# lvjiahui/DRT

Hardware: AMD Instinct MI355X
Metric: M camera-rays/s (forward+backward) on 50k-tri mesh, 72 views (higher is better)
Workload: dtype f32 traversal + f64 shading/gradients; 1 GPU; horse_vh.ply x4 (1 midpoint subdivision) = 50248 tris / 25126 verts, 72 turntable views, 1024x1024 rays/view, LBVH rebuilt every step, forward+ray_loss+backward+all-reduce+SGD; targets=horse_scan.ply, mode=dropin, hip_graph=False, outputs_recycled=True, ray_binding=True, views_per_gpu=72, views_per_call=72

## Files before the change

### drt_amd/csrc/drt_pipeline.hip

```cpp
#include "drt_device.h"
#include "drt_trace_kernel.h"
#include "drt_pathsink.h"


struct Ray64 {
    double* o;
    double* d;
};
struct Pipe {
    RayList r0, r1, r2;
    unsigned* count;
    unsigned* valid;
    int32_t* redo;
};




__device__ __forceinline__ void write_dead(int64_t i, double* out_ori, double* out_dir, uint8_t* mask, int32_t* face2) {
    const d3 z{0.0, 0.0, 0.0};
    store_d3(out_ori, i, z);
    store_d3(out_dir, i, z);
    mask[3 * i] = 0; mask[3 * i + 1] = 0; mask[3 * i + 2] = 0;
    face2[i] = -1;
// ... 15 lines not shown
        po[lane] = zero; pd[lane] = zero;
        if (lane < 32) { po[64 + lane] = zero; pd[64 + lane] = zero; }
        if (lane < 12) reinterpret_cast<F4*>(mask + 3 * i0)[lane] = zero;
        if (lane >= 16 && lane < 32) reinterpret_cast<F4*>(face2 + i0)[lane - 16] = ones;
    }
    if (lane >= 32 && lane < 48) reinterpret_cast<F4*>(face1 + i0)[lane - 32] = ones;
}

struct RasterIn {
    ViewModel* views;
    int mode;
    unsigned long long* zbuf;
    uint32_t* zmask;
    int32_t* gen_list;
    int img_w, img_h;
    int pending;
    int no_tree;
};
constexpr int32_t kFacePending = -2;

struct CullShared {
    unsigned tmp[kPathWaves + 1];
    uint8_t flag[kPathBlock];
    int slot[kPathBlock];
};

template <bool FUSED>
__device__ __forceinline__ void cull_patch(unsigned patch, bool prefilled, CullShared& sh, const Node4Q* __restrict__ nodes, int n_tris,
                                           const double* __restrict__ origin, const double* __restrict__ dir,
                                           const uint8_t* __restrict__ valid, int64_t n, double* __restrict__ out_ori,
                                           double* __restrict__ out_dir, uint8_t* __restrict__ mask,
                                           int32_t* __restrict__ face1, int32_t* __restrict__ face2, const Pipe& p, int tile_w, const RasterIn& rz) {
    unsigned* s_tmp = sh.tmp;
    uint8_t* s_flag = sh.flag;
    int* s_slot = sh.slot;
    const bool dead_writes = !FUSED && !prefilled;
    const int tid = threadIdx.x;
    const bool raster = rz.views != nullptr;
    const int vt = ((tid & 63) >> 4) * 64 + (tid >> 6) * 16 + (tid & 15);
    const unsigned patches_per_row = tile_w > 0 ? (unsigned)tile_w / 64u : 1u;
    {
        int64_t i = (int64_t)patch * kPathBlock + tid;
        unsigned y = 0, x = 0;
        if (tile_w > 0) {
            const unsigned prow = patch / patches_per_row;
            y = 4u * prow + (unsigned)(tid >> 6); x = 64u * (patch - prow * patches_per_row) + (unsigned)(tid & 63);
            i = (int64_t)y * tile_w + x;
        }
        if (raster && rz.mode == DRT_GRID_TRUST) {
            const unsigned view = y / (unsigned)rz.img_h;
            if (rz.views[view].ok && rz.views[view].all) {
                const int64_t row0 = i - (int64_t)(tid >> 6) * tile_w - (tid & 63);
                unsigned any = 0;
                for (int r = 0; r < 4; ++r) {
                    const int64_t g = (row0 + (int64_t)r * tile_w) >> 6;
                    any |= rz.zmask[g >> 5] >> (g & 31);
                }
                if (!(any & 1u)) {
                    if (dead_writes) write_dead_row<FUSED>(i - (tid & 63), tid & 63, out_ori, out_dir, mask, face1, face2);
                    return;
                }
            }
        }
        bool cand = false, generic = false;
        int32_t face = -1;
        unsigned clear_bit = 0;
        f3 o{0.f, 0.f, 0.f}, d{0.f, 0.f, 1.f};
        if (i < n) {
            unsigned long long key = kRasterEmpty;
            bool trusted = false;
            unsigned view = 0;
            if (raster) {
                view = y / (unsigned)rz.img_h;
                trusted = rz.mode == DRT_GRID_TRUST && rz.views[view].ok && rz.views[view].all;
                const unsigned word = rz.zmask[i >> 11], bit = 1u << ((i >> 6) & 31);
                if (word & bit) {
                    const int64_t zs = raster_slot(x, y, (unsigned)tile_w);
                    key = rz.zbuf[zs];
                    if (key != kRasterEmpty) rz.zbuf[zs] = kRasterEmpty;
                    clear_bit = bit;
                }
            }
            if (trusted) {
                if (key != kRasterEmpty && (!FUSED || valid[i])) {
                    o = to_f32(load_d3(origin, i)); d = to_f32(load_d3(dir, i));
                    cand = true;
                    face = (int32_t)(uint32_t)key;
                }
            } else if (!FUSED || valid[i]) {
                const d3 o64 = load_d3(origin, i), d64 = load_d3(dir, i);
                o = to_f32(o64); d = to_f32(d64);
                bool verified = false;
                if (raster) {
                    ViewModel& vm = rz.views[view];
                    verified = vm.ok && view_verify(vm, o64, d64, (double)x, (double)(y - view * (unsigned)rz.img_h));
                    if (!verified && vm.all) __hip_atomic_store(&vm.all, 0, __ATOMIC_RELAXED, __HIP_MEMORY_SCOPE_AGENT);
                }
                if (verified) {
                    cand = key != kRasterEmpty;
                    face = (int32_t)(uint32_t)key;
                } else {
                    cand = n_tris > 0 && (rz.no_tree || hits_top_boxes(nodes, o, d));
                    generic = cand;
                }
            } else if (raster && rz.mode == DRT_GRID_ESTABLISH) {
                ViewModel& vm = rz.views[view];
                if (vm.all && !(vm.ok && view_verify(vm, load_d3(origin, i), load_d3(dir, i), (double)x, (double)(y - view * (unsigned)rz.img_h))))
                    __hip_atomic_store(&vm.all, 0, __ATOMIC_RELAXED, __HIP_MEMORY_SCOPE_AGENT);
            }
        }
        const bool live = i < n;
        if (!dead_writes) {
        } else if (tile_w > 0 && __ballot(cand || !live) == 0ull) {
            write_dead_row<FUSED>(i - (tid & 63), tid & 63, out_ori, out_dir, mask, face1, face2);
        } else if (live && !cand) {
            face1[i] = -1;
            write_dead(i, out_ori, out_dir, mask, face2);
        }
        const int any_cand = __syncthreads_or(cand ? 1 : 0);
        if (clear_bit && (tid & 63) == 0) atomicAnd(&rz.zmask[i >> 11], ~clear_bit);
        if (!any_cand) return;
        int slot;
        if (tile_w > 0) {
            s_flag[vt] = cand ? 1 : 0;
            __syncthreads();
            s_slot[tid] = block_push(s_flag[tid] != 0, &p.count[0], s_tmp);
            __syncthreads();
            slot = s_slot[vt];
            __syncthreads();
        } else {
            slot = block_push(cand, &p.count[0], s_tmp);
        }
        if (slot >= 0) {
            p.r0.idx[slot] = (int32_t)i; store_ray32(p.r0.ray, slot, o, d);
            if (raster) p.r0.face[slot] = generic && rz.pending ? kFacePending : face;
        }
        if (raster && __syncthreads_or(generic ? 1 : 0)) {
            const int g = block_push(generic, &p.count[3], s_tmp);
            if (g >= 0) rz.gen_list[g] = slot;
        }
    }
}

template <bool FUSED>
__global__ void __launch_bounds__(kPathBlock, 8) k_cull(const Node4Q* __restrict__ nodes, int n_tris, const double* __restrict__ origin, const double* __restrict__ dir,
                                                      const uint8_t* __restrict__ valid, int64_t n, double* __restrict__ out_ori,
                                                      double* __restrict__ out_dir, uint8_t* __restrict__ mask,
                                                      int32_t* __restrict__ face1, int32_t* __restrict__ face2, Pipe p, int tile_w, RasterIn rz,
                                                      bool prefilled ) {
    __shared__ CullShared sh;
    cull_patch<FUSED>(blockIdx.x, prefilled, sh, nodes, n_tris, origin, dir, valid, n, out_ori, out_dir, mask, face1, face2, p, tile_w, rz);
}

struct StageFace {
    StageMem m;
    int32_t face[kStageCap];
};
template <bool FUSED>
__global__ void __launch_bounds__(kPathBlock) k_cull_listed(const uint32_t* __restrict__ patches, const unsigned* __restrict__ n_patches,
                                                           const Node4Q* __restrict__ nodes, int n_tris, const double* __restrict__ origin, const double* __restrict__ dir,
                                                           const uint8_t* __restrict__ valid, int64_t n, double* __restrict__ out_ori,
                                                           double* __restrict__ out_dir, uint8_t* __restrict__ mask,
                                                           int32_t* __restrict__ face1, int32_t* __restrict__ face2, Pipe p, int tile_w, RasterIn rz,
                                                           PathCtx c, bool direct, bool prefilled, Ray64 park) {
    __shared__ CullShared sh;
    __shared__ StageFace st;
    stage_init(st.m);
    const int tid = threadIdx.x, wave = tid >> 6, lane = tid & 63;
    const int vt = ((tid & 63) >> 4) * 64 + (tid >> 6) * 16 + (tid & 15);
    const unsigned ppr = (unsigned)tile_w / 64u;
    const RayList dst = direct ? p.r1 : p.r0;
    unsigned* const dst_count = direct ? &p.count[1] : &p.count[0];
    auto flush = [&]() {
        const unsigned cnt = st.m.n;
        if (tid == 0) st.m.base = cnt ? atomicAdd(dst_count, cnt) : 0u;
        __syncthreads();
        const unsigned base = st.m.base;
        for (unsigned k = tid; k < cnt; k += kPathBlock) { dst.idx[base + k] = st.m.idx[k]; if (!direct) dst.face[base + k] = st.face[k]; }
        for (unsigned k = tid; k < 6u * cnt; k += kPathBlock) dst.ray[6 * (int64_t)base + k] = st.m.ray[k];
        __syncthreads();
        if (tid == 0) st.m.n = 0u;
        __syncthreads();
    };
    unsigned n_hits = 0;
    const unsigned count = *n_patches;
    for (unsigned k = blockIdx.x; k < count; k += gridDim.x) {
        const unsigned patch = patches[k];
        const unsigned prow = patch / ppr;
        const unsigned y = 4u * prow + (unsigned)wave, x = 64u * (patch - prow * ppr) + (unsigned)lane;
        const unsigned view = y / (unsigned)rz.img_h;
        if (!(rz.views[view].ok && rz.views[view].all)) {
            cull_patch<FUSED>(patch, true, sh, nodes, n_tris, origin, dir, valid, n, out_ori, out_dir, mask, face1, face2, p, tile_w, rz);
            __syncthreads();
            continue;
        }
        const int64_t i = (int64_t)y * tile_w + x;
        unsigned long long key = kRasterEmpty;
        const unsigned word = rz.zmask[i >> 11], bit = 1u << ((i >> 6) & 31);
        if (word & bit) {
            const int64_t zs = raster_slot(x, y, (unsigned)tile_w);
            key = rz.zbuf[zs];
            if (key != kRasterEmpty) rz.zbuf[zs] = kRasterEmpty;
        }
        const bool cand = key != kRasterEmpty && (!FUSED || valid[i]);
        bool push = cand;
        f3 o{0.f, 0.f, 0.f}, d{0.f, 0.f, 1.f};
        if (cand) {
            if (direct) {
                const int32_t f1 = (int32_t)(uint32_t)key;
                face1[i] = f1;
                d3 v0, v1, v2;
                int32_t vid[3];
                Bounce b;
                load_tri64(c, f1, v0, v1, v2, vid);
                bounce_forward(load_d3(origin, i), load_d3(dir, i), v0, v1, v2, c.ior_ext, c.ior_int, b);
                push = !b.tir;
                o = to_f32(b.new_o); d = to_f32(b.wt);
                if (push && park.o) { store_d3(park.o, i, b.new_o); store_d3(park.d, i, b.wt); }
                if (!push && !FUSED) { if (prefilled) face2[i] = -1; else write_dead(i, out_ori, out_dir, mask, face2); }
                ++n_hits;
            } else {
                o = to_f32(load_d3(origin, i)); d = to_f32(load_d3(dir, i));
            }
        }
        sh.flag[vt] = push ? 1 : 0;
        __syncthreads();
        if ((word & bit) && lane == 0) atomicAnd(&rz.zmask[i >> 11], ~bit);
        const bool mine = sh.flag[tid] != 0;
        const unsigned long long bm = __ballot(mine);
        if (lane == 0) sh.tmp[wave] = (unsigned)__popcll(bm);
        __syncthreads();
        unsigned before = 0, tot = 0;
        for (int w = 0; w < kPathWaves; ++w) { const unsigned cw = sh.tmp[w]; if (w < wave) before += cw; tot += cw; }
        sh.slot[tid] = mine ? (int)(before + (unsigned)__popcll(bm & ((1ull << lane) - 1ull))) : -1;
        __syncthreads();
        if (push) {
            const unsigned slot = st.m.n + (unsigned)sh.slot[vt];
            st.m.idx[slot] = (int32_t)i;
            float* e = st.m.ray + 6 * slot;
            e[0] = o.x; e[1] = o.y; e[2] = o.z; e[3] = d.x; e[4] = d.y; e[5] = d.z;
            st.face[slot] = (int32_t)(uint32_t)key;
        }
        __syncthreads();
        if (tid == 0) st.m.n += tot;
        __syncthreads();
        if (st.m.n > kStageCap - kPathBlock) flush();
    }
    flush();
    if (direct) {
        unsigned h = n_hits;
        for (int off = 32; off >= 1; off >>= 1) h += __shfl_xor(h, off);
        if (lane == 0 && h) atomicAdd(&p.count[17], h);
    }
}

__global__ void __launch_bounds__(kPathBlock) k_patch_list(unsigned n_patches, int tile_w, RasterIn rz, uint32_t* __restrict__ list, unsigned* count) {
    __shared__ unsigned s_tmp[kPathWaves + 1];
    const unsigned patch = blockIdx.x * kPathBlock + threadIdx.x;
    bool take = false;
    if (patch < n_patches) {
        const unsigned ppr = (unsigned)tile_w / 64u, prow = patch / ppr;
        const unsigned view = (4u * prow) / (unsigned)rz.img_h;
        take = true;
        if (rz.views[view].ok && rz.views[view].all) {
            const int64_t row0 = (int64_t)(4u * prow) * tile_w + 64u * (patch - prow * ppr);
            unsigned any = 0;
            for (int r = 0; r < 4; ++r) {
                const int64_t g = (row0 + (int64_t)r * tile_w) >> 6;
                any |= rz.zmask[g >> 5] >> (g & 31);
            }
            take = (any & 1u) != 0;
        }
    }
    const int slot = block_push(take, count, s_tmp);
    if (slot >= 0) list[slot] = patch;
}

template <bool FUSED>
__global__ void __launch_bounds__(kPathBlock) k_shade1(PathCtx c, const double* __restrict__ origin, const double* __restrict__ dir,
                                                        double* __restrict__ out_ori, double* __restrict__ out_dir, uint8_t* __restrict__ mask,
                                                        int32_t* __restrict__ face1, int32_t* __restrict__ face2, Pipe p,
                                                        bool prefilled , Ray64 r64) {
    __shared__ StageMem stage;
    stage_init(stage);
    const unsigned n0 = p.count[0];
    const unsigned per_block = ((n0 + gridDim.x - 1) / gridDim.x + kPathBlock - 1) / kPathBlock * kPathBlock;
    const unsigned first = blockIdx.x * per_block, last = min(n0, first + per_block);
    for (unsigned base = first; base < last; base += kPathBlock) {
        const unsigned k = base + threadIdx.x;
        bool ok = false;
        int64_t i = 0;
        f3 o2{0.f, 0.f, 0.f}, d2{0.f, 0.f, 1.f};
        if (k < n0) {
            i = p.r0.idx[k];
            const int32_t f1 = p.r0.face[k];
            if (f1 != kFacePending) face1[i] = f1;
            if (f1 >= 0) {
                d3 v0, v1, v2;
                int32_t vid[3];
                Bounce b;
                load_tri64(c, f1, v0, v1, v2, vid);
                bounce_forward(load_d3(origin, i), load_d3(dir, i), v0, v1, v2, c.ior_ext, c.ior_int, b);
                ok = !b.tir;
                o2 = to_f32(b.new_o); d2 = to_f32(b.wt);
                if (ok && r64.o) { store_d3(r64.o, i, b.new_o); store_d3(r64.d, i, b.wt); }
            }
            if (!ok && !FUSED && f1 != kFacePending) { if (prefilled) face2[i] = -1; else write_dead(i, out_ori, out_dir, mask, face2); }
        }
        stage_push(stage, ok, (int32_t)i, o2, d2, p.r1, &p.count[1]);
    }
    stage_flush(stage, p.r1, &p.count[1]);
}

template <bool FUSED>
__global__ void __launch_bounds__(kTraceBlock) k_gen_late(PathCtx c, const double* __restrict__ origin, const double* __restrict__ dir,
                                                          double* __restrict__ out_ori, double* __restrict__ out_dir, uint8_t* __restrict__ mask,
                                                          int32_t* __restrict__ face1, int32_t* __restrict__ face2, Pipe p,
                                                          const int32_t* __restrict__ gen_list, bool prefilled, Ray64 r64) {
    __shared__ int32_t lds[kStackFast][kTraceBlock];
    const unsigned n = p.count[3];
    if (n == 0) return;
    Stack st = make_stack(lds, c.tc);
    for (unsigned k = blockIdx.x * kTraceBlock + threadIdx.x; k < n; k += gridDim.x * kTraceBlock) {
        const int32_t slot = gen_list[k];
        if (p.r0.face[slot] != kFacePending) continue;
        const int64_t i = p.r0.idx[slot];
        const float* e = p.r0.ray + 6 * (int64_t)slot;
        const Hit h = traverse<false>(c.tc.nodes, c.tc.tris, c.tc.n_tris, f3{e[0], e[1], e[2]}, f3{e[3], e[4], e[5]}, st);
        p.r0.face[slot] = h.face;
        face1[i] = h.face;
        bool ok = false;
        if (h.face >= 0) {
            d3 v0, v1, v2;
            int32_t vid[3];
            Bounce b;
            load_tri64(c, h.face, v0, v1, v2, vid);
            bounce_forward(load_d3(origin, i), load_d3(dir, i), v0, v1, v2, c.ior_ext, c.ior_int, b);
            ok = !b.tir;
            if (ok) {
                const unsigned s1 = atomicAdd(&p.count[1], 1u);
                p.r1.idx[s1] = (int32_t)i;
                store_ray32(p.r1.ray, (int)s1, to_f32(b.new_o), to_f32(b.wt));
                if (r64.o) { store_d3(r64.o, i, b.new_o); store_d3(r64.d, i, b.wt); }
            }
        }
        if (!ok && !FUSED) { if (prefilled) face2[i] = -1; else write_dead(i, out_ori, out_dir, mask, face2); }
    }
}

template <bool FUSED>
__global__ void __launch_bounds__(kPathBlock) k_shade2(PathCtx c, const double* __restrict__ origin, const double* __restrict__ dir,
                                                        double* __restrict__ out_ori, double* __restrict__ out_dir, uint8_t* __restrict__ mask,
                                                        const int32_t* __restrict__ face1, int32_t* __restrict__ face2, Pipe p,
                                                        bool parked ) {
    __shared__ StageMem stage;
    stage_init(stage);
    const unsigned n1 = p.count[1];
    const unsigned per_block = ((n1 + gridDim.x - 1) / gridDim.x + kPathBlock - 1) / kPathBlock * kPathBlock;
    const unsigned first = blockIdx.x * per_block, last = min(n1, first + per_block);
    for (unsigned base = first; base < last; base += kPathBlock) {
        const unsigned k = base + threadIdx.x;
        bool ok = false;
        int64_t i = 0;
        f3 o3{0.f, 0.f, 0.f}, d3f{0.f, 0.f, 1.f};
        if (k < n1) {
            i = p.r1.idx[k];
            const int32_t f2 = p.r1.face[k];
            if (f2 >= 0) {
                d3 v0, v1, v2;
                int32_t vid[3];
                Bounce b;
                d3 o2, d2;
                if (parked) {
                    o2 = load_d3(out_ori, i); d2 = load_d3(out_dir, i);
                } else {
                    load_tri64(c, face1[i], v0, v1, v2, vid);
                    bounce_forward(load_d3(origin, i), load_d3(dir, i), v0, v1, v2, c.ior_ext, c.ior_int, b);
                    o2 = b.new_o; d2 = b.wt;
                }
                load_tri64(c, f2, v0, v1, v2, vid);
                bounce_forward(o2, d2, v0, v1, v2, c.ior_ext, c.ior_int, b);
                ok = !b.tir;
                if (ok) {
                    o3 = to_f32(b.new_o); d3f = to_f32(b.wt);
                    face2[i] = f2;
                    if (!FUSED) {
                        store_d3(out_ori, i, b.new_o);
                        store_d3(out_dir, i, b.wt);
                        mask[3 * i] = 1; mask[3 * i + 1] = 1; mask[3 * i + 2] = 1;
                    }
                }
            }
            if (!ok) { if (FUSED) face2[i] = -1; else write_dead(i, out_ori, out_dir, mask, face2); }
        }
        stage_push(stage, ok, (int32_t)i, o3, d3f, p.r2, &p.count[2]);
    }
    stage_flush(stage, p.r2, &p.count[2]);
}

__global__ void __launch_bounds__(kPathBlock) k_finish(double* __restrict__ out_ori, double* __restrict__ out_dir, uint8_t* __restrict__ mask,
                                                        int32_t* __restrict__ face2, Pipe p, int64_t chunk_base, int32_t* __restrict__ valid_idx) {
    __shared__ StageMem stage;
    stage_init(stage);
    const RayList out{valid_idx, nullptr, nullptr};
    const unsigned n2 = p.count[2];
    const unsigned per_block = ((n2 + gridDim.x - 1) / gridDim.x + kPathBlock - 1) / kPathBlock * kPathBlock;
// ... 577 lines not shown

static int ensure_queues(drt_scene::Sub& w, int64_t n, bool fused, bool mega = false) {
    if (fused && mega && n > w.ray64_cap) {
        (void)hipFree(w.ray64); w.ray64 = nullptr; w.ray64_cap = 0;
        HIP_TRY(hipMalloc(&w.ray64, sizeof(double) * 6 * n));
        w.ray64_cap = n;
    }
    if (n > w.q_cap) {
        for (int k = 0; k < 3; ++k) {
            (void)hipFree(w.q_idx[k]); (void)hipFree(w.q_ray[k]); (void)hipFree(w.q_face[k]);
            w.q_idx[k] = nullptr; w.q_ray[k] = nullptr; w.q_face[k] = nullptr;
        }
        w.q_cap = 0;
        for (int k = 0; k < 3; ++k) {
            HIP_TRY(hipMalloc(&w.q_idx[k], sizeof(int32_t) * n));
            HIP_TRY(hipMalloc(&w.q_ray[k], sizeof(float) * 6 * n));
            HIP_TRY(hipMalloc(&w.q_face[k], sizeof(int32_t) * n));
        }
        (void)hipFree(w.redo); w.redo = nullptr;
        HIP_TRY(hipMalloc(&w.redo, sizeof(int32_t) * n));
        (void)hipFree(w.gen_list); w.gen_list = nullptr;
        HIP_TRY(hipMalloc(&w.gen_list, sizeof(int32_t) * n));
        w.q_cap = n;
    }
    if (fused && n > w.fused_cap) {
        (void)hipFree(w.tmp_face1); (void)hipFree(w.tmp_face2);
        w.tmp_face1 = w.tmp_face2 = nullptr; w.fused_cap = 0;
        HIP_TRY(hipMalloc(&w.tmp_face1, sizeof(int32_t) * n));
        HIP_TRY(hipMalloc(&w.tmp_face2, sizeof(int32_t) * n));
        w.fused_cap = n;
    }
    return DRT_OK;
}

static Pipe pipe_of(const drt_scene* s, const drt_scene::Sub& w) {
    return Pipe{RayList{w.q_idx[0], w.q_ray[0], w.q_face[0]}, RayList{w.q_idx[1], w.q_ray[1], w.q_face[1]},
                RayList{w.q_idx[2], w.q_ray[2], w.q_face[2]}, w.qcount, s->vcount, w.redo};
}

struct Plan { int64_t size; int count; int streams; };
static Plan plan_call(const drt_scene* s, int64_t n_rays, int tile_w, int tile_h) {
    int64_t unit = 256;
    if (tile_w >= 64 && tile_w % 64 == 0) unit = 4 * (int64_t)tile_w;
    if (unit > 256 && tile_h >= 4 && tile_h % 4 == 0 && n_rays % ((int64_t)tile_w * tile_h) == 0) unit = (int64_t)tile_w * tile_h;
    int64_t count = (n_rays + s->chunk_rays - 1) / s->chunk_rays;
    const int64_t by_min = n_rays / s->min_sub_rays;
    const int64_t most = (int64_t)s->n_sub * s->sub_per_stream;
    const int64_t want = by_min < most ? by_min : most;
    if (want > count) count = want;
    if (count < 1) count = 1;
    int64_t size = (n_rays + count - 1) / count;
    size = (size + unit - 1) / unit * unit;
    count = (n_rays + size - 1) / size;
    Plan pl;
    pl.size = size; pl.count = (int)count; pl.streams = count < s->n_sub ? (int)count : s->n_sub;
    if (s->prof_serial) pl.streams = 1;
    return pl;
}

__global__ void k_store_models(const ViewModel* __restrict__ work, ViewModel* __restrict__ cache, int n) {
    const int v = blockIdx.x * blockDim.x + threadIdx.x;
    if (v >= n) return;
    ViewModel m = work[v];
    m.all = (m.ok && m.all) ? 1 : 0;
    m.ok = m.all;
    cache[v] = m;
}

static bool raster_on(const drt_scene* s, int64_t n, int tile_w, int tile_h) {
    if (!s->use_raster || s->n_faces <= 0 || tile_w < 64 || tile_w % 64 != 0 || tile_h < 4 || tile_h % 4 != 0) return false;
    const int64_t image = (int64_t)tile_w * tile_h;
    return n > 0 && n % image == 0 && n / image <= 65535;
}

constexpr int kIntPreOri = 1 << 16, kIntPreDir = 1 << 17, kIntPreMask = 1 << 18, kIntMask = kIntPreOri | kIntPreDir | kIntPreMask;
extern "C++" {
template <bool FUSED>
static int launch_chunk(drt_scene* s, drt_scene::Sub& w, hipStream_t st, const PathCtx& pc, const Pipe& p, const double* o, const double* d, const uint8_t* valid,
                        int64_t n, double* out_ori, double* out_dir, uint8_t* mask, int32_t* face1, int32_t* face2, int tile_w, int tile_h,
                        int grid_mode, ViewModel* grid_cache ,
                        hipStream_t aux , int64_t chunk_base, int32_t* valid_idx,
                        bool* n_finished ,
                        int32_t* seed2 = nullptr ) {
    if (n_finished) *n_finished = false;
    const bool sparse_faces = (grid_mode & DRT_GRID_SPARSE_FACES) != 0;
    const bool pre_ori = (grid_mode & kIntPreOri) != 0, pre_dir = (grid_mode & kIntPreDir) != 0, pre_mask = (grid_mode & kIntPreMask) != 0;
    const bool all_verified = (grid_mode & DRT_GRID_ALL_VERIFIED) != 0 && (grid_mode & 3) == DRT_GRID_TRUST && grid_cache;
    grid_mode &= 3;
    const int gs = 8 * s->n_cu;
    if (tile_w < 64 || tile_w % 64 != 0 || n % (4 * (int64_t)tile_w) != 0) tile_w = 0;
    RasterIn rz{nullptr, 0, nullptr, nullptr, nullptr, 0, 0, 0, 0};
    const bool mega = s->mega_max_rays > 0 && n <= s->mega_max_rays && n_finished != nullptr;
    const Ray64 r64 = !mega ? Ray64{nullptr, nullptr} : (FUSED ? Ray64{w.ray64, w.ray64 + 3 * n} : Ray64{out_ori, out_dir});
    bool late_fill = false;
    hipStream_t fs = s->prof_serial ? st : s->build_stream;
    {
        hipStreamCaptureStatus cs = hipStreamCaptureStatusNone;
        if (fs != st && hipStreamIsCapturing(st, &cs) == hipSuccess && cs != hipStreamCaptureStatusNone) fs = aux ? aux : st;
    }
    const int64_t image = (int64_t)tile_w * tile_h;
    if (raster_on(s, n, tile_w, tile_h)) {
        const int n_views = (int)(n / image);
        int rc = ensure_raster(s, w, n, n_views, st);
        if (rc) return rc;
        if (!grid_cache) grid_mode = DRT_GRID_NONE;
        if (!FUSED && grid_mode == DRT_GRID_TRUST) {
            late_fill = s->fill_overlap;
            if (!late_fill) {
                StageTimer t(s, st, kStageFill);
                if (!pre_ori) (void)hipMemsetAsync(out_ori, 0, sizeof(double) * 3 * n, st);
                if (!pre_dir) (void)hipMemsetAsync(out_dir, 0, sizeof(double) * 3 * n, st);
                if (!pre_mask) (void)hipMemsetAsync(mask, 0, 3 * n, st);
            }
            if (!sparse_faces) { (void)hipMemsetAsync(face1, 0xFF, sizeof(int32_t) * n, st); (void)hipMemsetAsync(face2, 0xFF, sizeof(int32_t) * n, st); }
        }
        if (late_fill && mega) {
            if (fs != st && aux) fs = aux;
            if (fs != st) { HIP_TRY(hipEventRecord(w.fill_fork, st)); HIP_TRY(hipStreamWaitEvent(fs, w.fill_fork, 0)); }
            { StageTimer tf(s, fs, kStageFill);
              if (!pre_ori) (void)hipMemsetAsync(out_ori, 0, sizeof(double) * 3 * n, fs);
              if (!pre_dir) (void)hipMemsetAsync(out_dir, 0, sizeof(double) * 3 * n, fs);
              if (!pre_mask) (void)hipMemsetAsync(mask, 0, 3 * n, fs); }
            if (fs != st) HIP_TRY(hipEventRecord(w.fill_join, fs));
        }
        StageTimer t(s, st, kStageRaster);
        rc = launch_raster(s, w, st, o, d, n_views, tile_w, tile_h, grid_mode == DRT_GRID_TRUST ? grid_cache : nullptr);
        if (rc) return rc;
        rz = RasterIn{w.vmodel, grid_mode, w.zbuf, w.zmask, w.gen_list, tile_w, tile_h, all_verified ? 1 : 0, all_verified ? 1 : 0};
    }
    const bool pre_any = pre_ori || pre_dir || pre_mask;
    if (pre_any && !late_fill) HIP_TRY(hipStreamWaitEvent(st, s->prefill_done, 0));
    const bool tree_late = all_verified && rz.views != nullptr;
    if (!tree_late) { int rc = wait_build(s, st); if (rc) return rc; }
    const bool direct = s->cull_direct && rz.views && grid_mode == DRT_GRID_TRUST && !mega && n >= s->cull_direct_min_rays;
    const bool park = !FUSED && !mega && rz.views && grid_mode == DRT_GRID_TRUST && pre_ori && pre_dir && pre_mask && s->cull_park;
    const Ray64 r64p = park ? Ray64{out_ori, out_dir} : r64;
    if (park) HIP_TRY(hipStreamWaitEvent(st, s->prefill_done, 0));
    {
        int64_t* rc = s->route_counts;
        rc[kRouteTotal] += 1;
        rc[kRouteRaster] += rz.views != nullptr;
        rc[kRouteTrust] += rz.views && grid_mode == DRT_GRID_TRUST;
        rc[kRouteDirect] += direct;
        rc[kRoutePark] += park;
        rc[kRouteLateFill] += late_fill;
        rc[kRouteTreeLate] += tree_late;
        rc[kRouteMega] += mega;
    }
    { StageTimer t(s, st, kStageCull);
      const unsigned n_patches = (unsigned)((n + kPathBlock - 1) / kPathBlock);
      if (rz.views && grid_mode == DRT_GRID_TRUST) {
          uint32_t* list = reinterpret_cast<uint32_t*>(p.redo);
          k_patch_list<<<(n_patches + kPathBlock - 1) / kPathBlock, kPathBlock, 0, st>>>(n_patches, tile_w, rz, list, p.count + 7);
          k_cull_listed<FUSED><<<gs, kPathBlock, 0, st>>>(list, p.count + 7, pc.tc.nodes, pc.tc.n_tris, o, d, valid, n, out_ori, out_dir, mask, face1, face2, p, tile_w, rz,
                                                          pc, direct, late_fill, park ? Ray64{out_ori, out_dir} : Ray64{nullptr, nullptr});
      } else {
          k_cull<FUSED><<<n_patches, kPathBlock, 0, st>>>(pc.tc.nodes, pc.tc.n_tris, o, d, valid, n, out_ori, out_dir, mask, face1, face2, p, tile_w, rz,
                                                          pre_ori && pre_dir && pre_mask && sparse_faces);
      } }
    auto issue_late_fills = [&]() -> int {
        if (fs != st) { HIP_TRY(hipEventRecord(w.fill_fork, st)); HIP_TRY(hipStreamWaitEvent(fs, w.fill_fork, 0)); }
        { StageTimer tf(s, fs, kStageFill);
          if (!pre_ori) (void)hipMemsetAsync(out_ori, 0, sizeof(double) * 3 * n, fs);
          if (!pre_dir) (void)hipMemsetAsync(out_dir, 0, sizeof(double) * 3 * n, fs);
          if (!pre_mask) (void)hipMemsetAsync(mask, 0, 3 * n, fs); }
        if (fs != st) HIP_TRY(hipEventRecord(w.fill_join, fs));
        return DRT_OK;
    };
    const bool fills_after_shade1 = s->fill_after_shade1 && fs != st;
    if (late_fill && !mega && !fills_after_shade1) { int rc = issue_late_fills(); if (rc) return rc; }
    if (rz.views && grid_mode == DRT_GRID_ESTABLISH)
        k_store_models<<<(int)(n / ((int64_t)tile_w * tile_h) + 63) / 64, 64, 0, st>>>(w.vmodel, grid_cache, (int)(n / ((int64_t)tile_w * tile_h)));
    { StageTimer t(s, st, kStageTrace1);
      if (rz.views && all_verified) {
      } else if (rz.views) {
          const TraceOut out{p.r0.face, nullptr, nullptr, w.gen_list};
          launch_trace_list(kTraceClosestListed, s->grid_path, st, pc.tc, p.r0.ray, p.count + 3, out, p.redo, p.count + 4, p.count + 16, s->refill_min, s->inner_min, s->prof_stats ? s->prof_counts + kProfStages + 4 * 0 : nullptr);
      } else {
          launch_trace_list(kTraceClosest, s->grid_path, st, pc.tc, p.r0.ray, p.count + 0, TraceOut{p.r0.face, nullptr, nullptr, nullptr}, p.redo, p.count + 4, p.count + 16, s->refill_min, s->inner_min, s->prof_stats ? s->prof_counts + kProfStages + 4 * 0 : nullptr);
      } }
    if (mega) {
        if (late_fill && fs != st) HIP_TRY(hipStreamWaitEvent(st, w.fill_join, 0));
        if (pre_any) HIP_TRY(hipStreamWaitEvent(st, s->prefill_done, 0));
    }
    {
      StageTimer t(s, st, kStageShade1);
      k_shade1<FUSED><<<gs, kPathBlock, 0, st>>>(pc, o, d, out_ori, out_dir, mask, face1, face2, p, late_fill, r64p); }
    if (late_fill && !mega && fills_after_shade1) { int rc = issue_late_fills(); if (rc) return rc; }
    if (tree_late) {
        int rc = wait_build(s, st); if (rc) return rc;
        StageTimer t(s, st, kStageTrace1);
        k_gen_late<FUSED><<<kRedoGrid, kTraceBlock, 0, st>>>(pc, o, d, out_ori, out_dir, mask, face1, face2, p, w.gen_list, late_fill, r64p);
    }
    if (mega) {
        StageTimer t(s, st, kStagePath);
        k_path<FUSED><<<s->grid_mega, kPathBlock, 0, st>>>(pc, r64, out_ori, out_dir, mask, face2, p, p.count + 8, chunk_base, valid_idx,
                                                           s->mega_refill_min, s->inner_min, s->shade_min, s->prof_stats ? s->prof_counts + kProfStages + 4 * 1 : nullptr, s->prof_on);
        k_path_redo<FUSED><<<kRedoGrid, kTraceBlock, 0, st>>>(pc, o, d, face1, out_ori, out_dir, mask, face2, p, chunk_base, valid_idx);
        *n_finished = true;
        return DRT_OK;
    }
    { StageTimer t(s, st, kStageTrace2);
      unsigned long long* stats = s->prof_stats ? s->prof_counts + kProfStages + 4 * 1 : nullptr;
      if (seed2 && s->hit_seed)
          launch_trace_list(kTraceClosestSeeded, s->grid_path, st, pc.tc, p.r1.ray, p.count + 1, TraceOut{p.r1.face, nullptr, nullptr, nullptr}, p.redo, p.count + 5, p.count + 16, s->refill_min, s->inner_min, stats,
                                                                        TraceSeed{p.r1.idx, seed2, s->slot_of_face, tile_w > 0 && s->seed_tiled ? (unsigned)tile_w : 0u});
      else
          launch_trace_list(kTraceClosest, s->grid_path, st, pc.tc, p.r1.ray, p.count + 1, TraceOut{p.r1.face, nullptr, nullptr, nullptr}, p.redo, p.count + 5, p.count + 16, s->refill_min, s->inner_min, stats); }
    if (late_fill && fs != st) HIP_TRY(hipStreamWaitEvent(st, w.fill_join, 0));
    if (late_fill && pre_any) HIP_TRY(hipStreamWaitEvent(st, s->prefill_done, 0));
    { StageTimer t(s, st, kStageShade2);
      k_shade2<FUSED><<<gs, kPathBlock, 0, st>>>(pc, o, d, out_ori, out_dir, mask, face1, face2, p, park); }
    { StageTimer t(s, st, kStageTrace3);
      launch_trace_list(kTraceAny, s->grid_path, st, pc.tc, p.r2.ray, p.count + 2, TraceOut{p.r2.face, nullptr, nullptr, nullptr}, p.redo, p.count + 6, p.count + 16, s->refill_min, s->inner_min, s->prof_stats ? s->prof_counts + kProfStages + 4 * 2 : nullptr); }
    return DRT_OK;
}
}

static int fork_streams(drt_scene* s, hipStream_t st, int streams) {
    HIP_TRY(hipEventRecord(s->fork_ev, st));
    for (int k = 0; k < streams; ++k) HIP_TRY(hipStreamWaitEvent(s->sub[k].stream, s->fork_ev, 0));
    return DRT_OK;
}
static int join_streams(drt_scene* s, hipStream_t st, int streams) {
    for (int k = 0; k < streams; ++k) {
        HIP_TRY(hipEventRecord(s->sub[k].done, s->sub[k].stream));
        HIP_TRY(hipStreamWaitEvent(st, s->sub[k].done, 0));
    }
    return DRT_OK;
}

static ViewModel* sub_cache(void* d_grid_cache, int64_t b, int tile_w, int tile_h) {
    if (!d_grid_cache || tile_w <= 0 || tile_h <= 0) return nullptr;
    return static_cast<ViewModel*>(d_grid_cache) + b / ((int64_t)tile_w * tile_h);
}
static PathCtx sub_ctx(const drt_scene* s, const drt_scene::Sub& w, const double* d_verts, double ior_int, double ior_ext) {
    PathCtx pc = path_ctx(s, d_verts, ior_int, ior_ext);
    pc.tc.slow_stack = w.slow_stack;
    return pc;
}
#if defined(DRT_CHECK)
int check_counters_pipeline(unsigned long long* out4) { return read_check_counters(out4); }
#endif
int mega_blocks_per_cu() {
    int per_cu = 0;
    if (hipOccupancyMaxActiveBlocksPerMultiprocessor(&per_cu, k_path<false>, kPathBlock, 0) != hipSuccess || per_cu < 1) per_cu = 2;
    int f = 0;
    if (hipOccupancyMaxActiveBlocksPerMultiprocessor(&f, k_path<true>, kPathBlock, 0) == hipSuccess && f >= 1 && f < per_cu) per_cu = f;
    return per_cu;
}

static int32_t* take_seed(drt_scene* s, int64_t n_rays) {
    int32_t* p = s->seed.face2 && s->seed.n == n_rays ? s->seed.face2 : nullptr;
    s->seed = drt_scene::Seed{};
    return p;
}
static drt_scene::LossArm take_loss_arm(drt_scene* s, int64_t n_rays) {
    const drt_scene::LossArm a = s->loss_arm.loss && s->loss_arm.n == n_rays ? s->loss_arm : drt_scene::LossArm{};
    s->loss_arm = drt_scene::LossArm{};
    s->loss_taken = false;
    return a;
}

extern "C" {

int drt_render_seed(drt_scene_t* s, int32_t* d_seed_face2, int64_t n_rays) {
    CHECK_SCENE(s);
    if (n_rays < 0 || (d_seed_face2 == nullptr && n_rays != 0)) return fail(DRT_E_INVALID, "bad seed buffer");
    s->seed = drt_scene::Seed{d_seed_face2, n_rays};
    return DRT_OK;
}

int drt_render_loss_arm(drt_scene_t* s, const double* d_screen_pixel, const uint8_t* d_valid, double* d_loss, double* d_grad_verts, int64_t n_rays) {
    CHECK_SCENE(s);
    if (n_rays <= 0 || !d_screen_pixel || !d_valid || !d_loss || !d_grad_verts) return fail(DRT_E_INVALID, "drt_render_loss_arm: bad arguments");
    s->loss_arm = drt_scene::LossArm{d_screen_pixel, d_valid, d_loss, d_grad_verts, n_rays};
    return DRT_OK;
}

int drt_render_loss_taken(drt_scene_t* s) {
    return s && s->loss_taken ? 1 : 0;
}

static int flush_clean(drt_scene* s, hipStream_t st);
static int render_forward_impl(drt_scene_t* s, const double* d_verts, const double* d_origin, const double* d_dir, int64_t n_rays,
                               double ior_int, double ior_ext, double* d_out_ori, double* d_out_dir, uint8_t* d_mask,
                               int32_t* d_face1, int32_t* d_face2, int32_t* d_valid_idx, int64_t* d_n_valid, int tile_w, int tile_h,
                               int grid_mode, void* d_grid_cache, void* stream);
int drt_render_forward(drt_scene_t* s, const double* d_verts, const double* d_origin, const double* d_dir, int64_t n_rays,
                       double ior_int, double ior_ext, double* d_out_ori, double* d_out_dir, uint8_t* d_mask,
                       int32_t* d_face1, int32_t* d_face2, int32_t* d_valid_idx, int64_t* d_n_valid, int tile_w, int tile_h,
                       int grid_mode, void* d_grid_cache, void* stream) {
    hipStreamCaptureStatus cap0 = hipStreamCaptureStatusNone;
    const bool swap_ev = s && s->clean.rows && s->clean.captured && hipStreamIsCapturing((hipStream_t)stream, &cap0) == hipSuccess && cap0 != hipStreamCaptureStatusNone;
    if (swap_ev) std::swap(s->prefill_done, s->prefill_done_cap);
    const int rc = render_forward_impl(s, d_verts, d_origin, d_dir, n_rays, ior_int, ior_ext, d_out_ori, d_out_dir, d_mask, d_face1, d_face2, d_valid_idx,
                                       d_n_valid, tile_w, tile_h, grid_mode, d_grid_cache, stream);
    if (swap_ev) std::swap(s->prefill_done, s->prefill_done_cap);
    if (rc != DRT_OK && s) {
        s->clean = drt_scene::Clean{};
        s->n_prefill = 0;
        s->seed = drt_scene::Seed{};
        s->segs = drt_scene::Segs{};
        s->loss_arm = drt_scene::LossArm{};
        s->loss_taken = false;
    }
    return rc;
}
// ... 387 lines not shown
```

### drt_amd/csrc/drt_scene.h

```cpp
#pragma once
#include <hip/hip_runtime.h>

#include <cstdarg>
#include <cstdio>
#include <cstdlib>
#include <cstring>
#include <new>
#include <vector>

#include "../../include/drt_hip.h"
#include "drt_common.h"
#include "drt_closest.h"
#include "drt_edge.h"
#include "drt_fixed.h"
#include "drt_lbvh.h"
#include "drt_path.h"
#include "drt_raster.h"
#include "drt_shade.h"
#include "drt_traverse.h"
#include "drt_tri.h"

using namespace drt;


int fail(int code, const char* fmt, ...);
#define HIP_TRY(expr)                                                                         \
    do {                                                                                      \
        hipError_t e_ = (expr);                                                               \
        if (e_ != hipSuccess) return fail(DRT_E_HIP, "%s: %s", #expr, hipGetErrorString(e_)); \
    } while (0)

constexpr int kTraceBlock = 128;
#ifndef DRT_STACK_FAST
#define DRT_STACK_FAST 19
#endif
constexpr int kStackFast = DRT_STACK_FAST;
static_assert(kStackFast >= 3, "FastStack keeps four spare entries (kStackFast + 1 rows) above its usable depth");
constexpr int kStackTotal = 192;
constexpr int kStackSlowDev = kStackTotal - kStackFast;
constexpr int kQCount = 24;
constexpr int kRedoGrid = 64;
constexpr int kTraceGridMax = 4096;
constexpr int64_t kChunkRays = 1 << 26;

constexpr int kSortBlock = 256, kSortItems = 8, kSortTile = kSortBlock * kSortItems, kRadix = 256;

enum { kRouteTotal = 0, kRouteRaster, kRouteTrust, kRouteDirect, kRoutePark, kRouteLateFill, kRouteTreeLate, kRouteMega };
enum { kStageBuild = 0, kStageCull, kStageTrace1, kStageShade1, kStageTrace2, kStageShade2, kStageTrace3, kStageFinish, kStageCollect, kStageBackward, kStageLossBwdFused, kStageRaster, kStageFill, kStagePath, kProfStages };
static_assert(kProfStages == DRT_PROFILE_STAGES, "include/drt_hip.h");

struct BuildParams {
    float lox, loy, loz;
    float ix, iy, iz;
    float pad;
    int32_t reserved;
    MortonPlan plan;
};

struct drt_scene {
    int device = 0;
    int64_t n_faces = 0, n_verts = 0;
    int64_t cap_faces = 0, cap_verts = 0;
    int32_t* faces = nullptr;
    float* verts = nullptr;
    Node* nodes = nullptr;
    Node4Q* wide = nullptr;
    int32_t *range_lo = nullptr, *range_hi = nullptr;
    TriRec* tris = nullptr;
    TriRec* tris_flat = nullptr;
    int32_t* slot_of_face = nullptr;
    struct Seed { int32_t* face2 = nullptr; int64_t n = 0; } seed;
    struct LossArm { const double* screen_pixel = nullptr; const uint8_t* valid = nullptr; double* loss = nullptr; double* grad_verts = nullptr; int64_t n = 0; } loss_arm;
    bool loss_taken = false;
    hipStream_t build_stream = nullptr;
    hipEvent_t build_fork = nullptr, build_done = nullptr;
    bool build_pending = false;
    bool order_valid = false;
    int sorted_buf = 0;
    bool cull_direct = true;
    bool cull_park = true;
    int64_t cull_direct_min_rays = (int64_t)1 << 25;
    int64_t route_counts[8] = {0};
    int tree_mode = 0, rebuild_every = 1, since_full = 0;
    bool topology_fixed = false;
    uint32_t* bounds_acc = nullptr;
    bool async_build = true;
    uint32_t *keys[2] = {nullptr, nullptr}, *idx[2] = {nullptr, nullptr};
    uint32_t* hist = nullptr;
    int32_t *parent_inner = nullptr, *parent_leaf = nullptr;
    uint32_t* flags = nullptr;
    BuildParams* params = nullptr;
    int32_t* slow_stack = nullptr;
    unsigned long long* scratch = nullptr;
    int32_t *b1_list = nullptr, *b1_redo = nullptr;
    unsigned* b1_count = nullptr;
    int64_t b1_cap = 0;
    struct Sub {
        hipStream_t stream = nullptr;
        hipEvent_t done = nullptr;
        hipEvent_t tail = nullptr;
        hipEvent_t fill_fork = nullptr, fill_join = nullptr;
        int32_t* q_idx[3] = {nullptr, nullptr, nullptr};
        float* q_ray[3] = {nullptr, nullptr, nullptr};
        int32_t* q_face[3] = {nullptr, nullptr, nullptr};
        int32_t *tmp_face1 = nullptr, *tmp_face2 = nullptr;
        unsigned* qcount = nullptr;
        double* ray64 = nullptr;
        int64_t ray64_cap = 0;
        int32_t* redo = nullptr;
        int32_t* slow_stack = nullptr;
        int64_t q_cap = 0, fused_cap = 0;
        unsigned long long* zbuf = nullptr;
        uint32_t* zmask = nullptr;
        int64_t z_cap = 0;
        ViewModel* vmodel = nullptr;
        int vm_cap = 0;
        void* big = nullptr;
        unsigned* big_count = nullptr;
        int32_t* gen_list = nullptr;
    };
    static constexpr unsigned kBigCap = 1u << 20;
    static constexpr int kMaxSub = 4;
    Sub sub[kMaxSub];
    int n_sub = 2;
    int sub_per_stream = 1;
    int64_t min_sub_rays = 1 << 24;
    hipEvent_t fork_ev = nullptr;
    struct Clean { double* ori = nullptr; double* dir = nullptr; uint8_t* mask = nullptr; int64_t n = 0; const int32_t* rows = nullptr; const int64_t* n_rows = nullptr;
                   bool captured = false;  } clean;
    static constexpr int kMaxSeg = 32;
    unsigned* seg_counts = nullptr;
    struct Segs { const int32_t* list = nullptr; int n = 0; int stream0 = 0; } segs;
    struct Prefill { const void* ptr = nullptr; int64_t bytes = 0; };
    Prefill prefill[3];
    int n_prefill = 0;
    hipEvent_t prefill_fork = nullptr, prefill_done = nullptr, prefill_done_cap = nullptr;
    unsigned* vcount = nullptr;
    uint32_t* vh_list = nullptr;
    int64_t vh_cap = 0;
    bool prof_on = false;
    uint32_t prof_mask = ~0u;
    bool prof_stats = false;
    bool prof_serial = false;
    std::vector<hipEvent_t> prof_ev;
    std::vector<int> prof_stage;
    size_t prof_used = 0;
    size_t prof_dropped = 0;
    unsigned long long* prof_counts = nullptr;
    hipStream_t prof_stream = nullptr;
    int n_cu = 256;
    int grid_trace = 2048;
    int grid_path = 2048;
    int64_t trace_stats[12] = {0};
    int grid_mega = 1024;
    int64_t mega_max_rays = 0;
    int shade_min = 8;
    int mega_refill_min = 16;
    int refill_min = 32;
    int inner_min = 24;
    int64_t chunk_rays = kChunkRays;

    bool fill_after_shade1 = true;
    bool fill_overlap = true;
    bool grid_canary = true;
    unsigned canary_salt = 0;
    bool seed_tiled = true;
    bool arm_finish_beside = true;
    bool hit_seed = true;
    bool use_raster = true;
    bool built = false;
    void* paths_ws = nullptr;
    void* image_loss_ws = nullptr;
    void* image_views = nullptr;
};


int query_blocks_per_cu();
int pipeline_blocks_per_cu();
int mega_blocks_per_cu();

int ensure_raster(drt_scene* s, drt_scene::Sub& w, int64_t n_rays, int n_views, hipStream_t st);
int launch_raster(drt_scene* s, drt_scene::Sub& w, hipStream_t st, const double* d_origin, const double* d_dir, int n_views, int iw, int ih,
                  ViewModel* trusted);

void paths_free(drt_scene* s);
void image_loss_free(drt_scene* s);
void image_views_free(drt_scene* s);

int ensure_slow_stack(drt_scene* s, hipStream_t st);
bool det_mode();
#define DET_LAUNCH(kern, grid, block, st, ...)                                        \
    do {                                                                              \
        if (det_mode()) kern<true><<<grid, block, 0, st>>>(__VA_ARGS__);              \
// ... 65 lines not shown
```

Measured before the change: 43300 M camera-rays/s.

## Restructure listed cull into persistent batched blocks with atomic patch cursor

The listed cull kernel now launches a persistent grid sized from occupancy and CU count, and blocks grab runs of four patches through a global atomic cursor with prefetched next-run indices. It gathers candidate pixels into a shared batch first and runs the bounce and compaction once per batch, so there are fewer block-wide barriers and one global atomic per batch. Zbuf and zmask loads for a run of patches are issued together, the pixel-to-lane mapping is changed to 4x4 quads, and ray records are written as float2. Short lists use fewer active blocks. The counter block grows to hold the cursor word, and the cursor has to be reset between calls for this to stay correct.

Result: faster. 43950 M camera-rays/s (median of 6 runs) (+1.5%).

```diff
diff --git a/drt_amd/csrc/drt_pipeline.hip b/drt_amd/csrc/drt_pipeline.hip
--- a/drt_amd/csrc/drt_pipeline.hip
+++ b/drt_amd/csrc/drt_pipeline.hip
@@ -191,9 +191,18 @@
     cull_patch<FUSED>(blockIdx.x, prefilled, sh, nodes, n_tris, origin, dir, valid, n, out_ori, out_dir, mask, face1, face2, p, tile_w, rz);
 }
 
-struct StageFace {
-    StageMem m;
-    int32_t face[kStageCap];
+constexpr int kCullRun = 4;
+constexpr int kCullPer = kCullRun;
+constexpr int kCullCap = kCullRun * kPathBlock;
+constexpr int kCullCursor = 32;
+constexpr int kCullFewPerCu = 2;
+constexpr int kCullLongRuns = 16;
+static_assert(kCullCursor < kQCount, "the cursor word lies inside the counter block");
+struct CullBatch {
+    int32_t idx[kCullCap];
+    int32_t face[kCullCap];
+    unsigned n, base, next[2];
+    unsigned wtot[kCullPer][kPathWaves];
 };
 template <bool FUSED>
 __global__ void __launch_bounds__(kPathBlock) k_cull_listed(const uint32_t* __restrict__ patches, const unsigned* __restrict__ n_patches,
@@ -201,96 +210,161 @@
                                                            const uint8_t* __restrict__ valid, int64_t n, double* __restrict__ out_ori,
                                                            double* __restrict__ out_dir, uint8_t* __restrict__ mask,
                                                            int32_t* __restrict__ face1, int32_t* __restrict__ face2, Pipe p, int tile_w, RasterIn rz,
-                                                           PathCtx c, bool direct, bool prefilled, Ray64 park) {
+                                                           PathCtx c, bool direct, bool prefilled, Ray64 park, unsigned few, unsigned long_list) {
     __shared__ CullShared sh;
-    __shared__ StageFace st;
-    stage_init(st.m);
+    __shared__ CullBatch sb;
     const int tid = threadIdx.x, wave = tid >> 6, lane = tid & 63;
-    const int vt = ((tid & 63) >> 4) * 64 + (tid >> 6) * 16 + (tid & 15);
     const unsigned ppr = (unsigned)tile_w / 64u;
     const RayList dst = direct ? p.r1 : p.r0;
     unsigned* const dst_count = direct ? &p.count[1] : &p.count[0];
-    auto flush = [&]() {
-        const unsigned cnt = st.m.n;
-        if (tid == 0) st.m.base = cnt ? atomicAdd(dst_count, cnt) : 0u;
-        __syncthreads();
-        const unsigned base = st.m.base;
-        for (unsigned k = tid; k < cnt; k += kPathBlock) { dst.idx[base + k] = st.m.idx[k]; if (!direct) dst.face[base + k] = st.face[k]; }
-        for (unsigned k = tid; k < 6u * cnt; k += kPathBlock) dst.ray[6 * (int64_t)base + k] = st.m.ray[k];
-        __syncthreads();
-        if (tid == 0) st.m.n = 0u;
-        __syncthreads();
-    };
+    unsigned* const cursor = &p.count[kCullCursor];
     unsigned n_hits = 0;
     const unsigned count = *n_patches;
-    for (unsigned k = blockIdx.x; k < count; k += gridDim.x) {
-        const unsigned patch = patches[k];
-        const unsigned prow = patch / ppr;
-        const unsigned y = 4u * prow + (unsigned)wave, x = 64u * (patch - prow * ppr) + (unsigned)lane;
-        const unsigned view = y / (unsigned)rz.img_h;
-        if (!(rz.views[view].ok && rz.views[view].all)) {
-            cull_patch<FUSED>(patch, true, sh, nodes, n_tris, origin, dir, valid, n, out_ori, out_dir, mask, face1, face2, p, tile_w, rz);
-            __syncthreads();
-            continue;
-        }
-        const int64_t i = (int64_t)y * tile_w + x;
-        unsigned long long key = kRasterEmpty;
-        const unsigned word = rz.zmask[i >> 11], bit = 1u << ((i >> 6) & 31);
-        if (word & bit) {
-            const int64_t zs = raster_slot(x, y, (unsigned)tile_w);
-            key = rz.zbuf[zs];
-            if (key != kRasterEmpty) rz.zbuf[zs] = kRasterEmpty;
-        }
-        const bool cand = key != kRasterEmpty && (!FUSED || valid[i]);
-        bool push = cand;
-        f3 o{0.f, 0.f, 0.f}, d{0.f, 0.f, 1.f};
-        if (cand) {
-            if (direct) {
-                const int32_t f1 = (int32_t)(uint32_t)key;
-                face1[i] = f1;
-                d3 v0, v1, v2;
-                int32_t vid[3];
-                Bounce b;
-                load_tri64(c, f1, v0, v1, v2, vid);
-                bounce_forward(load_d3(origin, i), load_d3(dir, i), v0, v1, v2, c.ior_ext, c.ior_int, b);
-                push = !b.tir;
-                o = to_f32(b.new_o); d = to_f32(b.wt);
-                if (push && park.o) { store_d3(park.o, i, b.new_o); store_d3(park.d, i, b.wt); }
-                if (!push && !FUSED) { if (prefilled) face2[i] = -1; else write_dead(i, out_ori, out_dir, mask, face2); }
-                ++n_hits;
-            } else {
-                o = to_f32(load_d3(origin, i)); d = to_f32(load_d3(dir, i));
-            }
-        }
-        sh.flag[vt] = push ? 1 : 0;
+    const unsigned active = count >= long_list ? gridDim.x : min(few, gridDim.x);
+    if (blockIdx.x >= active) return;
+    unsigned first = blockIdx.x * (unsigned)kCullRun;
+    if (tid == 0) {
+        sb.n = 0u;
+        if (first < count) sb.next[0] = active * (unsigned)kCullRun + atomicAdd(cursor, (unsigned)kCullRun);
+    }
+    __syncthreads();
+
+    auto close_batch = [&]() {
+        const unsigned cnt = sb.n;
+        if (cnt == 0u) { __syncthreads(); return; }
+        int32_t ei[kCullPer], ef[kCullPer];
+        f3 eo[kCullPer], ed[kCullPer];
+        bool push[kCullPer];
+        unsigned rank[kCullPer];
+#pragma unroll
+        for (int j = 0; j < kCullPer; ++j) {
+            const unsigned k = (unsigned)(j * kPathBlock + tid);
+            push[j] = false;
+            ei[j] = 0; ef[j] = -1;
+            eo[j] = f3{0.f, 0.f, 0.f}; ed[j] = f3{0.f, 0.f, 1.f};
+            if (k < cnt) {
+                const int64_t i = sb.idx[k];
+                const int32_t f1 = sb.face[k];
+                ei[j] = (int32_t)i; ef[j] = f1;
+                if (direct) {
+                    face1[i] = f1;
+                    d3 v0, v1, v2;
+                    int32_t vid[3];
+                    Bounce b;
+                    load_tri64(c, f1, v0, v1, v2, vid);
+                    bounce_forward(load_d3(origin, i), load_d3(dir, i), v0, v1, v2, c.ior_ext, c.ior_int, b);
+                    push[j] = !b.tir;
+                    eo[j] = to_f32(b.new_o); ed[j] = to_f32(b.wt);
+                    if (push[j] && park.o) { store_d3(park.o, i, b.new_o); store_d3(park.d, i, b.wt); }
+                    if (!push[j] && !FUSED) { if (prefilled) face2[i] = -1; else write_dead(i, out_ori, out_dir, mask, face2); }
+                    ++n_hits;
+                } else {
+                    eo[j] = to_f32(load_d3(origin, i)); ed[j] = to_f32(load_d3(dir, i));
+                    push[j] = true;
+                }
+            }
+            const unsigned long long bm = __ballot(push[j]);
+            if (lane == 0) sb.wtot[j][wave] = (unsigned)__popcll(bm);
+            rank[j] = (unsigned)__popcll(bm & ((1ull << lane) - 1ull));
+        }
         __syncthreads();
-        if ((word & bit) && lane == 0) atomicAnd(&rz.zmask[i >> 11], ~bit);
-        const bool mine = sh.flag[tid] != 0;
-        const unsigned long long bm = __ballot(mine);
-        if (lane == 0) sh.tmp[wave] = (unsigned)__popcll(bm);
+        unsigned tot = 0;
+#pragma unroll
+        for (int j = 0; j < kCullPer; ++j) {
+            unsigned before = tot;
+#pragma unroll
+            for (int w = 0; w < kPathWaves; ++w) { const unsigned cw = sb.wtot[j][w]; if (w < wave) before += cw; tot += cw; }
+            rank[j] += before;
+        }
+        if (tid == 0) { sb.base = tot ? atomicAdd(dst_count, tot) : 0u; sb.n = 0u; }
         __syncthreads();
-        unsigned before = 0, tot = 0;
-        for (int w = 0; w < kPathWaves; ++w) { const unsigned cw = sh.tmp[w]; if (w < wave) before += cw; tot += cw; }
-        sh.slot[tid] = mine ? (int)(before + (unsigned)__popcll(bm & ((1ull << lane) - 1ull))) : -1;
+        const unsigned base = sb.base;
+#pragma unroll
+        for (int j = 0; j < kCullPer; ++j) {
+            if (!push[j]) continue;
+            const unsigned slot = base + rank[j];
+            dst.idx[slot] = ei[j];
+            float2* e = reinterpret_cast<float2*>(dst.ray + 6 * (int64_t)slot);
+            e[0] = float2{eo[j].x, eo[j].y}; e[1] = float2{eo[j].z, ed[j].x}; e[2] = float2{ed[j].y, ed[j].z};
+            if (!direct) dst.face[slot] = ef[j];
+        }
+    };
+
+    for (unsigned it = 0; first < count; ++it) {
+        const unsigned cnt = min((unsigned)kCullRun, count - first);
+        uint32_t pt[kCullRun];
+        bool ok[kCullRun];
+        unsigned word[kCullRun];
+        unsigned long long key[kCullRun];
+        int64_t zs[kCullRun], ri[kCullRun];
+#pragma unroll
+        for (int j = 0; j < kCullRun; ++j) pt[j] = (unsigned)j < cnt ? patches[first + j] : 0u;
+#pragma unroll
+        for (int j = 0; j < kCullRun; ++j) {
+            const unsigned prow = pt[j] / ppr;
+            const unsigned x = 64u * (pt[j] - prow * ppr) + 16u * (unsigned)wave + 4u * ((unsigned)lane >> 4) + ((unsigned)lane & 3u);
+            const unsigned y = 4u * prow + (((unsigned)lane >> 2) & 3u);
+            const unsigned view = (4u * prow) / (unsigned)rz.img_h;
+            ri[j] = (int64_t)y * tile_w + x;
+            zs[j] = raster_slot(x, y, (unsigned)tile_w);
+            ok[j] = false; word[j] = 0u; key[j] = kRasterEmpty;
+            if ((unsigned)j < cnt) {
+                ok[j] = rz.views[view].ok && rz.views[view].all;
+                word[j] = rz.zmask[ri[j] >> 11];
+                key[j] = rz.zbuf[zs[j]];
+            }
+        }
+#pragma unroll
+        for (int j = 0; j < kCullRun; ++j) {
+            if ((unsigned)j >= cnt) continue;
+            if (!ok[j]) {
+                cull_patch<FUSED>(pt[j], true, sh, nodes, n_tris, origin, dir, valid, n, out_ori, out_dir, mask, face1, face2, p, tile_w, rz);
+                __syncthreads();
+                continue;
+            }
+            const int64_t i = ri[j];
+            const bool has = ((word[j] >> ((i >> 6) & 31)) & 1u) != 0u && key[j] != kRasterEmpty;
+            if (has) rz.zbuf[zs[j]] = kRasterEmpty;
+            const bool take = has && (!FUSED || valid[i]);
+            const unsigned long long bm = __ballot(take);
+            if (bm != 0ull) {
+                unsigned at = 0u;
+                if (lane == 0) at = atomicAdd(&sb.n, (unsigned)__popcll(bm));
+                at = (unsigned)__shfl((int)at, 0);
+                if (take) {
+                    const unsigned k = at + (unsigned)__popcll(bm & ((1ull << lane) - 1ull));
+                    sb.idx[k] = (int32_t)i;
+                    sb.face[k] = (int32_t)(uint32_t)key[j];
+                }
+            }
+        }
         __syncthreads();
-        if (push) {
-            const unsigned slot = st.m.n + (unsigned)sh.slot[vt];
-            st.m.idx[slot] = (int32_t)i;
-            float* e = st.m.ray + 6 * slot;
-            e[0] = o.x; e[1] = o.y; e[2] = o.z; e[3] = d.x; e[4] = d.y; e[5] = d.z;
-            st.face[slot] = (int32_t)(uint32_t)key;
-        }
-        __syncthreads();
-        if (tid == 0) st.m.n += tot;
-        __syncthreads();
-        if (st.m.n > kStageCap - kPathBlock) flush();
-    }
-    flush();
+        if (tid < 4 * (int)cnt) {
+            const unsigned q = patches[first + ((unsigned)tid >> 2)], prow = q / ppr;
+            const int64_t i0 = (int64_t)(4u * prow + ((unsigned)tid & 3u)) * tile_w + 64u * (q - prow * ppr);
+            const unsigned bit = 1u << ((i0 >> 6) & 31);
+            if (rz.zmask[i0 >> 11] & bit) atomicAnd(&rz.zmask[i0 >> 11], ~bit);
+        }
+        const unsigned nxt = sb.next[it & 1u];
+        if (tid == 0 && nxt < count) sb.next[(it + 1u) & 1u] = active * (unsigned)kCullRun + atomicAdd(cursor, (unsigned)kCullRun);
+        close_batch();
+        first = nxt;
+    }
     if (direct) {
         unsigned h = n_hits;
         for (int off = 32; off >= 1; off >>= 1) h += __shfl_xor(h, off);
         if (lane == 0 && h) atomicAdd(&p.count[17], h);
     }
+}
+constexpr int kCullSgprBlocks = 6;
+int cull_blocks_per_cu() {
+    int per_cu = 0;
+    if (hipOccupancyMaxActiveBlocksPerMultiprocessor(&per_cu, k_cull_listed<false>, kPathBlock, 0) != hipSuccess || per_cu < 1) per_cu = 4;
+    int f = 0;
+    if (hipOccupancyMaxActiveBlocksPerMultiprocessor(&f, k_cull_listed<true>, kPathBlock, 0) == hipSuccess && f >= 1 && f < per_cu) per_cu = f;
+    if (per_cu > 8) per_cu = 8;
+    if (per_cu > kCullSgprBlocks) per_cu = kCullSgprBlocks;
+    return per_cu;
 }
 
 __global__ void __launch_bounds__(kPathBlock) k_patch_list(unsigned n_patches, int tile_w, RasterIn rz, uint32_t* __restrict__ list, unsigned* count) {
@@ -1174,8 +1248,10 @@
       if (rz.views && grid_mode == DRT_GRID_TRUST) {
           uint32_t* list = reinterpret_cast<uint32_t*>(p.redo);
           k_patch_list<<<(n_patches + kPathBlock - 1) / kPathBlock, kPathBlock, 0, st>>>(n_patches, tile_w, rz, list, p.count + 7);
-          k_cull_listed<FUSED><<<gs, kPathBlock, 0, st>>>(list, p.count + 7, pc.tc.nodes, pc.tc.n_tris, o, d, valid, n, out_ori, out_dir, mask, face1, face2, p, tile_w, rz,
-                                                          pc, direct, late_fill, park ? Ray64{out_ori, out_dir} : Ray64{nullptr, nullptr});
+          static const int cull_per_cu = cull_blocks_per_cu();
+          const unsigned few = (unsigned)(kCullFewPerCu * s->n_cu), long_list = few * (unsigned)(kCullRun * kCullLongRuns);
+          k_cull_listed<FUSED><<<cull_per_cu * s->n_cu, kPathBlock, 0, st>>>(list, p.count + 7, pc.tc.nodes, pc.tc.n_tris, o, d, valid, n, out_ori, out_dir, mask, face1, face2, p, tile_w, rz,
+                                                          pc, direct, late_fill, park ? Ray64{out_ori, out_dir} : Ray64{nullptr, nullptr}, few, long_list);
       } else {
           k_cull<FUSED><<<n_patches, kPathBlock, 0, st>>>(pc.tc.nodes, pc.tc.n_tris, o, d, valid, n, out_ori, out_dir, mask, face1, face2, p, tile_w, rz,
                                                           pre_ori && pre_dir && pre_mask && sparse_faces);
diff --git a/drt_amd/csrc/drt_scene.h b/drt_amd/csrc/drt_scene.h
--- a/drt_amd/csrc/drt_scene.h
+++ b/drt_amd/csrc/drt_scene.h
@@ -38,7 +38,7 @@
 static_assert(kStackFast >= 3, "FastStack keeps four spare entries (kStackFast + 1 rows) above its usable depth");
 constexpr int kStackTotal = 192;
 constexpr int kStackSlowDev = kStackTotal - kStackFast;
-constexpr int kQCount = 24;
+constexpr int kQCount = 64;
 constexpr int kRedoGrid = 64;
 constexpr int kTraceGridMax = 4096;
 constexpr int64_t kChunkRays = 1 << 26;
```
